# awslabs/flowgger

Hardware: NVIDIA H100
Metric: log lines/sec parsed (RFC5424) (higher is better)
Workload: dtype u8

## Files before the change

### flowgger_b200/csrc/fg_abi.cu

```cuda
#include <cuda_runtime.h>

#include <algorithm>
#include <chrono>
#include <cstdio>
#include <cstdlib>
#include <cstring>
#include <ctime>
#include <mutex>
#include <new>
#include <string>
#include <utility>
#include <vector>

#include "../../include/flowgger_cuda.h"
#include "fg_kernels.cuh"
#include "fg_status.h"
#include "fg_rfc3164.cuh"
#include "fg_tz.h"

namespace {

const char* kErrorStrings[FG_ST_COUNT] = {};
struct ErrorTableInit {
    ErrorTableInit() {
// ... 90 lines not shown
    H h = nullptr;
    Handle() = default;
    Handle(Handle&& o) noexcept : h(o.h) { o.h = nullptr; }
    Handle(const Handle&) = delete;
    Handle& operator=(const Handle&) = delete;
    ~Handle() {
        if (h) destroy(h);
    }
    operator H() const { return h; }
};
using Event = Handle<cudaEvent_t>;
using Stream = Handle<cudaStream_t>;

struct StepEvents {
    Event h2d;
    Event k0, k1;
    Event cnt;
};

enum { T_ENTRIES, T_E8, T_ARENA, T_WIDE, T_COUNT };
struct TableShape {
    size_t width[3];
    size_t round;
};
constexpr TableShape kTableShape[T_COUNT] = {
    {{sizeof(fg_span), sizeof(uint64_t), 1}, 256},
    {{sizeof(uint64_t), 0, 0}, 256},
    {{1, 0, 0}, 256},
    {{sizeof(fg_wide_row), 0, 0}, 1},
};
static_assert(sizeof(fg_span) == sizeof(int2) && sizeof(fg_wide_row) == sizeof(fg::WideRow), "pinned rows mirror the device rows");
struct Table {
    Buf<uint8_t> col[3];
    size_t cap = 0;
};

struct TableUse {
    int table, counter;
    size_t div, floor;
    bool grow;
};
struct FormatTables {
    int n;
    TableUse use[4];
    const TableUse* begin() const { return use; }
    const TableUse* end() const { return use + n; }
};
constexpr FormatTables kFormatTables[4] = {
    {4, {{T_E8, fg::K5_ENTRIES, 24, 4096, false}, {T_ARENA, fg::K5_ARENA, 64, 64 << 10, false},
         {T_WIDE, fg::K5_WIDE_ROWS, 0, 1024, false}, {T_ENTRIES, fg::K5_WIDE_ENTRIES, 0, 4096, false}}},
    {1, {{T_ENTRIES, fg::K5_ENTRIES, 24, 4096, true}}},
    {1, {{T_ENTRIES, fg::K5_ENTRIES, 24, 4096, true}}},
    {2, {{T_ARENA, fg::K5_ARENA, 32, 64 << 10, false}, {T_ENTRIES, -1, 0, 256, false}}},
};

}

struct fg_ctx {
    int device = 0;
    size_t max_bytes = 0;
    int max_lines = 0;
    int chunk_lines = 0;
    int input_format = 0;
    Stream s_h2d, s_comp, s_d2h;
    Stream s_parse;
    Event ev_a, ev_b;
    Event ev_dom0, ev_dom1;
    Event ev_s0, ev_s1;
    std::vector<StepEvents> steps;
    std::vector<Event> ev_split;
    Event bounce_ev[2];
    Buf<uint8_t> bounce[2];
    Buf<uint32_t> counts;
    Buf<uint8_t> bytes;
    Buf<int32_t> offsets;
    Buf<uint32_t> k;
    Buf<uint8_t> flush;
    Table tab[T_COUNT];
    Buf<uint8_t> rows;
    Buf<int2> tmp_name;
    Buf<unsigned long long> tmp_val;
    Buf<uint8_t> tmp_meta;
    Buf<fg::Row5424, fg_row5424> rows5;
    Buf<uint32_t> esc_list, wide_list;
    Buf<unsigned long long> enc_lens, enc_rel;
    Buf<unsigned long long> enc_base;
    Buf<uint8_t> enc_out;
    size_t enc_out_cap = 0;
    Buf<long long, int64_t> enc_offsets;
    Buf<uint8_t> enc_status;
    Buf<int32_t> enc_stop;
    int enc_stop_n = -1;
    Buf<uint8_t> scan_temp;
    size_t scan_temp_bytes = 0;
    Buf<uint8_t> static_blob;
    int n_static = 0;
    const int32_t* d_static_key_off = nullptr;
    const int32_t* d_static_lit_off = nullptr;
    const int32_t* d_static_kind = nullptr;
    std::vector<std::pair<std::string, std::string>> gelf_extra;
    Buf<uint32_t> seg;
    Buf<int32_t> n_lines;
    Buf<uint8_t> invalid;
    Buf<int32_t> split_offsets;
    Buf<int32_t> cum;
    float last_split_ms = 0.f;
    int r3164_year = 0;
    int call_year = 1970;
    std::string tzdir;
    fg::TzHostTable tz_host;
    Buf<uint8_t> tz_blob;
    fg::TzDeviceTable tz_dev{};
    Buf<uint8_t> ltsv_blob;
    fg::LtsvDeviceConfig ltsv{};
    float last_dom_ms = 0.f;
    int res_n = 0;
    size_t res_bytes = 0;
    int res_fmt = -1;
    uint32_t res_tot[fg::K5_COUNT] = {};
    std::string last_error;
    int64_t launches = 0;
    int max_tile5 = 0;
    int num_sms = 0;
};

namespace {

constexpr int kColW[9] = {8, 4, 8, 8, 8, 8, 8, 8, 8};
enum { C_TS = 0, C_META, C_HOST, C_APP, C_PROC, C_MSGID, C_MSG, C_FULL, C_SD, C_COUNT };
size_t col_off(const fg_ctx* c, int col) {
    const size_t n = (size_t)c->max_lines;
    size_t o = 0;
    for (int k = 0; k < col; ++k) o += (size_t)kColW[k] * n;
    return o;
}

int fail(fg_ctx* c, int code, const char* what, cudaError_t e = cudaSuccess) {
    if (c) {
        c->last_error = what;
        if (e != cudaSuccess) {
            c->last_error += ": ";
            c->last_error += cudaGetErrorString(e);
        }
    }
    return code;
}

#define FG_CUDA(ctx, call)                                         \
    do {                                                           \
        cudaError_t _e = (call);                                   \
        if (_e != cudaSuccess) return fail(ctx, FG_E_CUDA, #call, _e); \
    } while (0)

cudaError_t create(Event& e, unsigned flags) { return cudaEventCreateWithFlags(&e.h, flags); }
cudaError_t create(Stream& s) { return cudaStreamCreateWithFlags(&s.h, cudaStreamNonBlocking); }

template <class T>
T* dev(const fg_ctx* c, int t, int col = 0) {
    return reinterpret_cast<T*>(c->tab[t].col[col].d);
}
template <class T>
T* host(const fg_ctx* c, int t, int col = 0) {
    return reinterpret_cast<T*>(c->tab[t].col[col].h);
}
uint32_t cap32(const fg_ctx* c, int t) { return (uint32_t)std::min<size_t>(c->tab[t].cap, 0xFFFFFFFFu); }

int grow_table(fg_ctx* c, int t, size_t rows) {
// ... 38 lines not shown
    std::vector<uint8_t> bytes;
    template <class V>
    size_t add(const V& v) {
        const size_t at = bytes.size();
        const uint8_t* src = reinterpret_cast<const uint8_t*>(v.data());
        bytes.insert(bytes.end(), src, src + v.size() * sizeof(v[0]));
        bytes.resize((bytes.size() + 15) & ~(size_t)15, 0);
        return at;
    }
    int upload(fg_ctx* c, Buf<uint8_t>& blob) {
        bytes.resize(bytes.size() + 16, 0);
        FG_CUDA(c, blob.alloc(bytes.size(), DEV));
        FG_CUDA(c, cudaMemcpy(blob.d, bytes.data(), bytes.size(), cudaMemcpyHostToDevice));
        return FG_OK;
    }
};

int upload_tz(fg_ctx* c) {
    const fg::TzHostTable& H = c->tz_host;
    Packer p;
    const size_t o_hash = p.add(H.hash), o_key = p.add(H.key), o_zone = p.add(H.zone), o_noff = p.add(H.name_off),
                 o_first = p.add(H.first), o_off = p.add(H.off), o_names = p.add(H.names);
    if (int rc = p.upload(c, c->tz_blob)) return rc;
    const uint8_t* b = c->tz_blob.d;
    fg::TzDeviceTable& T = c->tz_dev;
    T = H.view();
    T.hash = (const unsigned long long*)(b + o_hash);
    T.key = (const long long*)(b + o_key);
    T.zone = (const int32_t*)(b + o_zone);
    T.name_off = (const int32_t*)(b + o_noff);
    T.first = (const int32_t*)(b + o_first);
    T.off = (const int32_t*)(b + o_off);
    T.names = b + o_names;
    return FG_OK;
}

int upload_ltsv_config(fg_ctx* c, const fg_config* cfg) {
    std::vector<uint8_t> names, suffix;
    std::vector<int32_t> name_off{0}, types;
    const int ns = (cfg->ltsv_schema_names && cfg->ltsv_schema_types) ? cfg->ltsv_schema_len : 0;
    for (int k = 0; k < ns; ++k) {
        const char* s = cfg->ltsv_schema_names[k];
        names.insert(names.end(), (const uint8_t*)s, (const uint8_t*)s + strlen(s));
        name_off.push_back((int32_t)names.size());
        types.push_back(cfg->ltsv_schema_types[k]);
    }
    fg::LtsvDeviceConfig& L = c->ltsv;
    L.has_schema = (cfg->ltsv_has_schema || ns > 0) ? 1 : 0;
    L.n_schema = ns;
    L.suffix_present = 0;
    L.suffix_off[0] = 0;
    for (int t = 0; t < 5; ++t) {
        const char* s = cfg->ltsv_suffix[t];
        if (t > 0 && s) {
            L.suffix_present |= 1u << t;
            suffix.insert(suffix.end(), (const uint8_t*)s, (const uint8_t*)s + strlen(s));
        }
        L.suffix_off[t + 1] = (int32_t)suffix.size();
    }
    Packer p;
    const size_t o_names = p.add(names), o_off = p.add(name_off), o_types = p.add(types), o_suf = p.add(suffix);
    if (int rc = p.upload(c, c->ltsv_blob)) return rc;
    const uint8_t* b = c->ltsv_blob.d;
    L.names = b + o_names;
    L.name_off = (const int32_t*)(b + o_off);
    L.types = (const int32_t*)(b + o_types);
    L.suffix = b + o_suf;
    return FG_OK;
}

int current_year(const fg_ctx* c) {
    if (c->r3164_year != 0) return c->r3164_year;
    const time_t now = time(nullptr);
    struct tm g;
    gmtime_r(&now, &g);
    return g.tm_year + 1900;
}

int ensure_format(fg_ctx* c, int fmt) {
    const size_t L = (size_t)c->max_lines;
    if (fmt == FG_FMT_RFC5424) {
        if (!c->rows5.d) {
            FG_CUDA(c, c->rows5.alloc(L, BOTH));
            FG_CUDA(c, c->esc_list.alloc(L, DEV));
            FG_CUDA(c, c->wide_list.alloc(L, DEV));
        }
    } else if (!c->rows.d) {
        FG_CUDA(c, c->rows.alloc(col_off(c, C_COUNT), BOTH));
    }
    if (fmt == FG_FMT_GELF && !c->wide_list.d) FG_CUDA(c, c->wide_list.alloc(L, DEV));
    for (const TableUse& u : kFormatTables[fmt]) {
        const size_t first = u.div ? std::max<size_t>(c->max_bytes / u.div, u.floor) : u.floor;
        const size_t cap = c->tab[u.table].cap;
        if (u.grow ? cap < first : !cap)
            if (int rc = grow_table(c, u.table, first)) return rc;
    }
    if (fmt == FG_FMT_RFC3164) {
        if (!c->tz_host.loaded) {
            std::string err;
            if (!fg::tz_load_dir(c->tzdir.empty() ? nullptr : c->tzdir.c_str(), c->tz_host, err)) return fail(c, FG_E_ARG, err.c_str());
        }
        if (!c->tz_blob.d)
            if (int rc = upload_tz(c)) return rc;
    }
    if (fmt == FG_FMT_LTSV || fmt == FG_FMT_GELF) {
        const size_t need = (fmt == FG_FMT_LTSV ? c->max_bytes / 2 + L : c->max_bytes / 3) + 64;
        if (c->tmp_meta.n < need) {
            c->tmp_name.reset(); c->tmp_val.reset(); c->tmp_meta.reset();
            FG_CUDA(c, c->tmp_name.alloc(need, DEV));
            FG_CUDA(c, c->tmp_val.alloc(need, DEV));
            FG_CUDA(c, c->tmp_meta.alloc(need, DEV));
        }
    }
    return FG_OK;
}

int begin_call(fg_ctx* c, fg_format fmt) {
    if ((int)fmt < 0 || (int)fmt > 3) return fail(c, FG_E_ARG, "unknown format");
    FG_CUDA(c, cudaSetDevice(c->device));
    if (int rc = ensure_format(c, (int)fmt)) return rc;
    c->call_year = current_year(c);
    return FG_OK;
}

int pick_tile(const fg_ctx* c, size_t total_bytes, int n, int fmt) {
    const double mean = n > 0 ? (double)total_bytes / n : 0.0;
    const long lines = fg::lines_per_cta(fmt), gran = 8 * lines;
    const int max_tile[4] = {c->max_tile5, fg::kLtsvMaxTile, fg::kGelfMaxTile, fg::kR3164MaxTile};
    long t = (long)(mean * lines * 1.02) + gran;
    t = (t + gran - 1) / gran * gran;
    t = std::max(t, 8L * 1024);
    t = std::min(t, (long)max_tile[fmt]);
    return (int)t;
}

int launch_lines(fg_ctx* c, int fmt, int line0, int n, int tile, const uint8_t* invalid, int strip_eol, cudaStream_t s,
                 bool time_dominant = false) {
    if (fmt == FG_FMT_RFC5424) {
        fg::Parse5424Params P;
        P.bytes = c->bytes.d;
        P.offsets = c->offsets.d + line0;
        P.n = n;
        P.tile_bytes = tile;
        P.rows = reinterpret_cast<uint4*>(c->rows5.d + line0);
        P.entries = dev<unsigned long long>(c, T_E8);
        P.entry_cap = cap32(c, T_E8);
        P.counters = c->k.d;
        P.esc_list = c->esc_list.d;
        P.wide_list = c->wide_list.d;
        P.arena = dev<uint8_t>(c, T_ARENA);
        P.arena_cap = cap32(c, T_ARENA);
        P.wide_rows = dev<fg::WideRow>(c, T_WIDE);
        P.wide_cap = cap32(c, T_WIDE);
        P.wentry_name = dev<int2>(c, T_ENTRIES, 0);
        P.wentry_val = dev<unsigned long long>(c, T_ENTRIES, 1);
        P.wentry_meta = dev<uint8_t>(c, T_ENTRIES, 2);
        P.wentry_cap = cap32(c, T_ENTRIES);
        P.line0 = line0;
        P.bad_offsets = c->k.d + fg::K5_BAD_OFFSETS;
        P.line_invalid = invalid;
        P.strip_eol = strip_eol;
        P.num_sms = c->num_sms;
        FG_CUDA(c, cudaMemsetAsync(c->k.d + fg::K5_ESC_LIST, 0, 8, s));
        FG_CUDA(c, fg::launch_parse5424(P, s, time_dominant ? c->ev_dom0.h : nullptr, time_dominant ? c->ev_dom1.h : nullptr));
        c->launches += 2;
        return FG_OK;
    }
    fg::ParseParams P;
    P.bytes = c->bytes.d;
    P.offsets = c->offsets.d + line0;
    P.n = n;
    P.line0 = line0;
    P.tile_bytes = tile;
    P.num_sms = c->num_sms;
    uint8_t* r = c->rows.d;
    P.ts = (double*)(r + col_off(c, C_TS)) + line0;
    P.meta = (uint32_t*)(r + col_off(c, C_META)) + line0;
    P.host = (int2*)(r + col_off(c, C_HOST)) + line0;
    P.app = (int2*)(r + col_off(c, C_APP)) + line0;
    P.proc = (int2*)(r + col_off(c, C_PROC)) + line0;
    P.msgid = (int2*)(r + col_off(c, C_MSGID)) + line0;
    P.msg = (int2*)(r + col_off(c, C_MSG)) + line0;
    P.full = (int2*)(r + col_off(c, C_FULL)) + line0;
    P.sd = (int2*)(r + col_off(c, C_SD)) + line0;
    P.entry_name = dev<int2>(c, T_ENTRIES, 0);
    P.entry_val = dev<unsigned long long>(c, T_ENTRIES, 1);
    P.entry_meta = dev<uint8_t>(c, T_ENTRIES, 2);
    P.tmp_name = c->tmp_name.d;
    P.tmp_val = c->tmp_val.d;
    P.tmp_meta = c->tmp_meta.d;
    P.line_invalid = invalid;
    P.strip_eol = strip_eol;
    P.entry_counter = c->k.d + fg::K5_ENTRIES;
    P.entry_cap = cap32(c, T_ENTRIES);
    P.bad_offsets = c->k.d + fg::K5_BAD_OFFSETS;
    P.slow_list = c->wide_list.d;
    P.slow_count = c->k.d + fg::K5_WIDE_LIST;
    if (fmt == FG_FMT_GELF) FG_CUDA(c, cudaMemsetAsync(c->k.d + fg::K5_WIDE_LIST, 0, 4, s));
    P.ltsv = c->ltsv;
    P.r3164.year = c->call_year;
    P.r3164.tz = c->tz_dev;
    P.r3164.arena = dev<uint8_t>(c, T_ARENA);
    P.r3164.arena_cap = cap32(c, T_ARENA);
    P.r3164.arena_counter = c->k.d + fg::K5_ARENA;
    if (time_dominant) FG_CUDA(c, cudaEventRecord(c->ev_dom0, s));
    FG_CUDA(c, fg::launch_parse(fmt, P, s));
    if (time_dominant) FG_CUDA(c, cudaEventRecord(c->ev_dom1, s));
    c->launches += fmt == FG_FMT_GELF ? 2 : 1;
    return FG_OK;
}

bool gelf_fusable(const fg_ctx* c, int fmt) {
    return fmt == FG_FMT_RFC5424 || fmt == FG_FMT_RFC3164 || (fmt == FG_FMT_LTSV && c->input_format == FG_FMT_LTSV);
}

int launch_encode(fg_ctx* c, int fmt, int k, int l0, int n, int tile, cudaStream_t s) {
    fg::GelfEncodeParams E{};
    E.bytes = c->bytes.d;
    E.offsets = c->offsets.d + l0;
    E.n = n;
    if (fmt == FG_FMT_RFC5424) {
        E.rows = reinterpret_cast<const uint4*>(c->rows5.d + l0);
    } else {
        const uint8_t* r = c->rows.d;
        E.col_ts = (const double*)(r + col_off(c, C_TS)) + l0;
        E.col_meta = (const uint32_t*)(r + col_off(c, C_META)) + l0;
        E.col_host = (const int2*)(r + col_off(c, C_HOST)) + l0;
        E.col_msg = (const int2*)(r + col_off(c, C_MSG)) + l0;
        E.col_full = (const int2*)(r + col_off(c, C_FULL)) + l0;
    }
    if (fmt == FG_FMT_LTSV) {
        E.col_sd = (const int2*)(c->rows.d + col_off(c, C_SD)) + l0;
        E.ltsv_suffix = c->ltsv.suffix;
        for (int t = 0; t < 6; ++t) E.ltsv_suffix_off[t] = c->ltsv.suffix_off[t];
        E.ltsv_stop = c->enc_stop.d + l0;
    }
    E.entries = dev<unsigned long long>(c, T_E8);
    E.arena = dev<uint8_t>(c, T_ARENA);
    E.wide_rows = dev<fg::WideRow>(c, T_WIDE);
    E.wentry_name = dev<int2>(c, T_ENTRIES, 0);
    E.wentry_val = dev<unsigned long long>(c, T_ENTRIES, 1);
    E.wentry_meta = dev<uint8_t>(c, T_ENTRIES, 2);
    E.static_blob = c->static_blob.d;
    E.n_static = c->n_static;
    E.static_key_off = c->d_static_key_off;
    E.static_lit_off = c->d_static_lit_off;
// ... 855 lines not shown
```

### flowgger_b200/csrc/fg_kernels.cuh

```cuda
#pragma once
#include <stdint.h>
#ifdef FG_HOST_EMU
#include "../../tests/emu/cuda_shim.h"
#else
#include <cuda_runtime.h>
#endif

namespace fg {

struct LtsvDeviceConfig {
    int32_t has_schema;
    int32_t n_schema;
    const uint8_t* names;
    const int32_t* name_off;
    const int32_t* types;
    const uint8_t* suffix;
    int32_t suffix_off[6];
    uint32_t suffix_present;
};

struct TzDeviceTable {
    int32_t n_names;
    int32_t min_len, max_len;
    uint32_t first_mask[8];
    const unsigned long long* hash;
    const int32_t* zone;
    const int32_t* name_off;
    const uint8_t* names;
    const int32_t* first;
    const long long* key;
    const int32_t* off;
};
struct R3164DeviceConfig {
    int32_t year;
    TzDeviceTable tz;
    uint8_t* arena;
    uint32_t arena_cap;
    uint32_t* arena_counter;
};

struct ParseParams {
    const uint8_t* bytes;
    const int32_t* offsets;
    int32_t n;
    int32_t line0;
    int32_t tile_bytes;
    double* ts;
    uint32_t* meta;
    int2* host;
    int2* app;
    int2* proc;
    int2* msgid;
    int2* msg;
    int2* full;
    int2* sd;
    int2* entry_name;
    unsigned long long* entry_val;
    uint8_t* entry_meta;
    int2* tmp_name;
    unsigned long long* tmp_val;
    uint8_t* tmp_meta;
    const uint8_t* line_invalid;
    int32_t strip_eol;
    uint32_t* entry_counter;
    uint32_t entry_cap;
    const uint32_t* bad_offsets;
    uint32_t* slow_list;
    uint32_t* slow_count;
    int32_t num_sms;
    LtsvDeviceConfig ltsv;
    R3164DeviceConfig r3164;
};

struct Row5424 {
    double ts;
    uint32_t meta;
    uint32_t sd_first;
    uint16_t sd_count;
    uint16_t sp[5];
    uint16_t msg_off, msg_len;
};
static_assert(sizeof(Row5424) == 32, "Row5424 must be 32 bytes");
struct WideRow {
    int32_t line;
    uint32_t meta;
    double ts;
    int2 host, app, proc, msgid, msg, full, sd;
};
static_assert(sizeof(WideRow) == 72, "WideRow must be 72 bytes");

enum { K5_ENTRIES = 0, K5_ARENA = 1, K5_WIDE_ROWS = 2, K5_WIDE_ENTRIES = 3, K5_ESC_LIST = 4, K5_WIDE_LIST = 5, K5_BAD_OFFSETS = 6,
       K5_COUNT = 8 };

struct Parse5424Params {
    const uint8_t* bytes;
    const int32_t* offsets;
    int32_t n;
    int32_t tile_bytes;
    uint4* rows;
    unsigned long long* entries;
    uint32_t entry_cap;
    uint32_t* counters;
    uint32_t* esc_list;
    uint32_t* wide_list;
    uint8_t* arena;
    uint32_t arena_cap;
    WideRow* wide_rows;
    uint32_t wide_cap;
    int2* wentry_name;
    unsigned long long* wentry_val;
    uint8_t* wentry_meta;
    uint32_t wentry_cap;
    int32_t line0;
    const uint32_t* bad_offsets;
    const uint8_t* line_invalid;
    int32_t strip_eol;
    int32_t num_sms;
};

cudaError_t launch_parse5424(const Parse5424Params& p, cudaStream_t stream, cudaEvent_t dom0 = nullptr, cudaEvent_t dom1 = nullptr);
cudaError_t configure_parse5424(int max_tile_bytes);
int parse5424_smem_bytes(int tile_bytes);

struct GelfEncodeParams {
    const uint8_t* bytes;
    const int32_t* offsets;
    int32_t n;
    const uint4* rows;
    const unsigned long long* entries;
    const uint8_t* arena;
    const WideRow* wide_rows;
    const int2* wentry_name;
    const unsigned long long* wentry_val;
    const uint8_t* wentry_meta;
    const uint8_t* static_blob;
    int32_t n_static;
    const int32_t* static_key_off;
    const int32_t* static_lit_off;
    const int32_t* static_kind;
    unsigned long long* lens;
    unsigned long long* rel;
    unsigned long long* base;
    uint8_t* out;
    unsigned long long out_cap;
    long long* out_offsets;
    uint8_t* status;
    const uint32_t* bad_offsets;
    uint32_t entry_cap, wide_cap, wentry_cap;
    int32_t tile_bytes;
    const double* col_ts;
    const uint32_t* col_meta;
    const int2* col_host;
    const int2* col_msg;
    const int2* col_full;
    uint32_t arena_cap;
    const int2* col_sd;
    const uint8_t* ltsv_suffix;
    int32_t ltsv_suffix_off[6];
    int32_t* ltsv_stop;
};
cudaError_t configure_gelf_encode(int max_tile_bytes);
cudaError_t launch_gelf_encode(int fmt, const GelfEncodeParams& p, void* d_scan_temp, size_t scan_temp_bytes, cudaStream_t stream);
size_t gelf_scan_temp_bytes(int n);

#ifndef FG_R5_LINES
#define FG_R5_LINES 64
#endif
#ifndef FG_R5_MINB
#define FG_R5_MINB 16
#endif
constexpr int kRfc5424LinesPerCta = FG_R5_LINES;
constexpr int kRfc5424CtasPerSm = FG_R5_MINB;
#ifndef FG_LTSV_LINES
#define FG_LTSV_LINES 64
#endif
#ifndef FG_LTSV_THREADS
#define FG_LTSV_THREADS 256
#endif
constexpr int kLtsvLinesPerCta = FG_LTSV_LINES;
constexpr int kLtsvThreadsPerCta = FG_LTSV_THREADS;
constexpr int kLtsvStageSlots = kLtsvLinesPerCta * 24;
constexpr int kLtsvMaxTile = 65024;
#ifndef FG_GELF_LINES
#define FG_GELF_LINES 64
#endif
#ifndef FG_GELF_THREADS
// ... 43 lines not shown
```

### flowgger_b200/csrc/fg_parse5424.cu

```cuda
#include "fg_kernels.cuh"

#include "fg_common.cuh"
#include "fg_r5fast.cuh"
#include "fg_rfc5424.cuh"
#include "fg_status.h"
#include "fg_tma.cuh"

namespace fg {

namespace {

constexpr int kFastLines = kRfc5424LinesPerCta;
constexpr int kFastCtasPerSm = kRfc5424CtasPerSm;

template <int LINES, int MINB>
__global__ void __launch_bounds__(LINES, MINB) parse5424_kernel(const __grid_constant__ Parse5424Params P) {
    extern __shared__ __align__(128) uint8_t tile[];
    __shared__ __align__(8) uint64_t mbar;
    __shared__ uint32_t scan_ws[2 * (LINES / 32)];
    __shared__ uint32_t s_base[3];

    const int tid = threadIdx.x;
    const uint32_t lane = (uint32_t)tid & 31u;
    const int first = blockIdx.x * LINES;
    const int last = min(P.n, first + LINES);
    uint32_t* bmI = reinterpret_cast<uint32_t*>(tile + P.tile_bytes);
    if (*P.bad_offsets) return;
    if (tid == 0) mbar_init(&mbar, 1);
    __syncthreads();

    uint32_t parity = 0;
    int cur = first;
    while (cur < last) {
        const int i = cur + tid;
        const int o0 = __ldg(P.offsets + min(i, last));
        const int o1 = __ldg(P.offsets + min(i + 1, last));
        const int ocur = __ldg(P.offsets + cur);
        const int base = ocur & ~15;
        const bool fits = (i < last) && (o1 - base <= P.tile_bytes);
        const int r = __syncthreads_count(fits);
        if (r == 0) {
            if (tid == 0) P.wide_list[atomicAdd(P.counters + K5_WIDE_LIST, 1u)] = (uint32_t)cur;
            cur += 1;
            continue;
        }
        const int oend = __ldg(P.offsets + cur + r);
        const uint32_t nbytes = (uint32_t)((oend - base) + 15) & ~15u;
        if (tid == 0) {
            fence_proxy_async();
            mbar_expect_tx(&mbar, nbytes);
            bulk_g2s(tile, P.bytes + base, nbytes, &mbar);
        }
        mbar_wait(&mbar, parity);
        parity ^= 1u;

        const int nword = (int)((nbytes + 31u) >> 5);
        for (int g = tid; g < nword; g += LINES) {
            const uint4 v0 = reinterpret_cast<const uint4*>(tile)[2 * g], v1 = reinterpret_cast<const uint4*>(tile)[2 * g + 1];
            bmI[g] = r5_classify16(v0.x, v0.y, v0.z, v0.w) | (r5_classify16(v1.x, v1.y, v1.z, v1.w) << 16);
        }
        if (tid < 3) bmI[nword + tid] = 0;
        __syncthreads();

        const bool active = tid < r;
        int ls = active ? o0 - base : 0;
        int le = active ? o1 - base : 0;
        bool bad_utf8 = false;
        if (P.strip_eol && le > ls) {
            if (P.strip_eol == 2) {
                if (tile[le - 1] == 0) --le;
            } else if (tile[le - 1] == '\n') {
                --le;
                if (le > ls && tile[le - 1] == '\r') --le;
            }
            if (P.line_invalid != nullptr && P.line_invalid[i]) bad_utf8 = true;
        }
        const bool too_long = le - ls > 65535;
        R5Fast res;
        const bool regular = r5_regular(tile, bmI, ls, (too_long || bad_utf8 || !active) ? ls : le, res);
        if (bad_utf8) {
            res.status = FG_ES_INVALID_UTF8;
            res.n_entries = 0;
        }
        const bool wide = active && !regular && !bad_utf8;
        const uint32_t my_n = (active && !wide && res.status == FG_ST_OK) ? res.n_entries : 0u;
        const bool esc = my_n != 0u && res.esc;

        uint32_t xa = my_n, xb = (esc ? 1u : 0u) | (wide ? 0x100u : 0u);
#pragma unroll
        for (int d = 1; d < 32; d <<= 1) {
            const uint32_t ya = __shfl_up_sync(0xFFFFFFFFu, xa, d), yb = __shfl_up_sync(0xFFFFFFFFu, xb, d);
            if (lane >= (uint32_t)d) { xa += ya; xb += yb; }
        }
        const int wid = tid >> 5;
        constexpr int kWarps = LINES / 32;
        if (lane == 31u) { scan_ws[wid] = xa; scan_ws[kWarps + wid] = xb; }
        __syncthreads();
        uint32_t before_a = 0, before_b = 0, total = 0, total_b = 0;
#pragma unroll
        for (int w = 0; w < kWarps; ++w) {
            const uint32_t ta = scan_ws[w], tb = scan_ws[kWarps + w];
            if (w < wid) { before_a += ta; before_b += tb; }
            total += ta;
            total_b += tb;
        }
        const uint32_t excl = before_a + xa - my_n;
        const uint32_t pos_b = before_b + xb - ((esc ? 1u : 0u) | (wide ? 0x100u : 0u));
        const uint32_t n_esc = total_b & 0xFFu, n_wide = total_b >> 8;
        if (total | total_b) {
            if (tid == 0 && total) s_base[0] = atomicAdd(P.counters + K5_ENTRIES, total);
            if (tid == 32 % LINES && n_esc) s_base[1] = atomicAdd(P.counters + K5_ESC_LIST, n_esc);
            if (tid == 33 % LINES && n_wide) s_base[2] = atomicAdd(P.counters + K5_WIDE_LIST, n_wide);
            __syncthreads();
        }
        const uint32_t esc_at = pos_b & 0xFFu, wide_at = pos_b >> 8;
        uint32_t my_begin = 0;
        if (my_n) {
            my_begin = s_base[0] + excl;
            if ((unsigned long long)my_begin + my_n <= (unsigned long long)P.entry_cap) {
                unsigned long long* dst = P.entries + my_begin;
                for (uint32_t k = 0; k < my_n; ++k) dst[k] = res.stage[k];
            }
        }
        if (esc) P.esc_list[s_base[1] + esc_at] = (uint32_t)i;
        if (wide) P.wide_list[s_base[2] + wide_at] = (uint32_t)i;
        if (active && !wide) {
            const bool ok = res.status == FG_ST_OK;
            const uint32_t meta = ok ? (res.facility << 8) | (res.severity << 16) | (res.flags << 24) : res.status | 0x00FFFF00u;
            uint4 lo4, hi4;
            lo4.x = (uint32_t)__double2loint(res.ts);
            lo4.y = (uint32_t)__double2hiint(res.ts);
            lo4.z = meta;
            lo4.w = my_begin;
            hi4.x = my_n | ((uint32_t)res.sp1 << 16);
            hi4.y = (uint32_t)res.sp2 | ((uint32_t)res.sp3 << 16);
            hi4.z = (uint32_t)res.sp4 | ((uint32_t)res.sp5 << 16);
            hi4.w = (uint32_t)res.msg_o | ((uint32_t)res.msg_l << 16);
            if (!ok) {
                lo4.x = lo4.y = 0u;
                hi4 = make_uint4(0u, 0u, 0u, 0u);
            }
            P.rows[2 * (size_t)i] = lo4;
            P.rows[2 * (size_t)i + 1] = hi4;
        }
        __syncthreads();
        cur += r;
    }
}

__device__ __forceinline__ void unescape_lines(const Parse5424Params& P, uint32_t first_item, uint32_t stride) {
    const uint32_t cnt = P.counters[K5_ESC_LIST];
    const uint32_t lane = threadIdx.x & 31u;
    for (uint32_t j0 = first_item; j0 < cnt; j0 += stride) {
        const uint32_t j = j0 + lane;
        const bool valid = j < cnt;
        uint32_t first = 0, count = 0;
        int o0 = 0;
        if (valid) {
            const uint32_t line = P.esc_list[j];
            const uint4 lo4 = P.rows[2 * (size_t)line], hi4 = P.rows[2 * (size_t)line + 1];
            o0 = P.offsets[line];
            first = lo4.w;
            count = hi4.x & 0xFFFFu;
            if ((unsigned long long)first + count > (unsigned long long)P.entry_cap) count = 0;
        }
        uint32_t need = 0;
        for (uint32_t e = 0; e < count; ++e) {
            const unsigned long long v = P.entries[first + e];
            if (!(v & kE8Header) && (v & kE8Esc)) need += (2u + (uint32_t)((v >> 32) & 0xFFFFu) - ((uint32_t)((v >> 16) & 0xFFFFu) + 2u) + 1u) & ~1u;
        }
        uint32_t inc = need;
#pragma unroll
        for (int d = 1; d < 32; d <<= 1) {
            const uint32_t y = __shfl_up_sync(0xFFFFFFFFu, inc, d);
            if (lane >= (uint32_t)d) inc += y;
        }
        const uint32_t warp_total = __shfl_sync(0xFFFFFFFFu, inc, 31);
        uint32_t abase = 0;
        if (lane == 0 && warp_total) abase = atomicAdd(P.counters + K5_ARENA, warp_total);
        abase = __shfl_sync(0xFFFFFFFFu, abase, 0);
        if ((unsigned long long)abase + warp_total > (unsigned long long)P.arena_cap) continue;
        uint32_t at = abase + inc - need;
        uint32_t e = 0;
        for (;;) {
            unsigned long long v = 0;
            bool have = false;
            for (; e < count; ++e) {
                v = P.entries[first + e];
                if (!(v & kE8Header) && (v & kE8Esc)) { have = true; break; }
            }
            if (!__any_sync(0xFFFFFFFFu, have)) break;
            const int ne = (int)((v >> 16) & 0xFFFFu), ve = (int)((v >> 32) & 0xFFFFu);
            const int len = have ? ve - (ne + 2) : 0;
            const uint8_t* src = P.bytes + o0 + ne + 2;
            uint8_t* dst = P.arena + at + 2;
            int k = 0, o = 0;
            while (__any_sync(0xFFFFFFFFu, k < len)) {
                if (k < len) {
                    const uint32_t c = src[k++];
                    if (c != '\\') {
                        dst[o++] = (uint8_t)c;
                    } else if (k < len) {
                        const uint32_t d = src[k++];
                        if (d != '"' && d != '\\' && d != ']') dst[o++] = '\\';
                        dst[o++] = (uint8_t)d;
                    }
                }
            }
            if (have) {
                *reinterpret_cast<uint16_t*>(P.arena + at) = (uint16_t)o;
                P.entries[first + e] = (v & 0xFFFFFFFFull) | ((unsigned long long)(at >> 1) << 32) | kE8Arena;
                at += (2u + (uint32_t)len + 1u) & ~1u;
                ++e;
            }
        }
    }
}

__device__ __forceinline__ void wide_lines(const Parse5424Params& P, int (*marks)[32], uint32_t first_item, uint32_t stride) {
    const uint32_t cnt = P.counters[K5_WIDE_LIST];
    const uint32_t lane = threadIdx.x & 31u;
    const EntrySink sink = {P.wentry_name, P.wentry_val, P.wentry_meta};
    for (uint32_t j0 = first_item; j0 < cnt; j0 += stride) {
        const uint32_t j = j0 + lane;
        const bool valid = j < cnt;
        uint32_t line = 0;
        int o0 = 0, len = 0;
        bool bad_utf8 = false;
        if (valid) {
            line = P.wide_list[j];
            o0 = P.offsets[line];
            len = P.offsets[line + 1] - o0;
            if (P.strip_eol && len > 0) {
                if (P.strip_eol == 2) {
                    if (P.bytes[o0 + len - 1] == 0) --len;
                } else if (P.bytes[o0 + len - 1] == '\n') {
                    --len;
                    if (len > 0 && P.bytes[o0 + len - 1] == '\r') --len;
                }
                if (P.line_invalid != nullptr && P.line_invalid[line]) bad_utf8 = true;
            }
            if (bad_utf8) len = 0;
        }
        LineResult res;
        rfc5424_parse_line<32>(P.bytes + o0, len, o0, &marks[0][lane], res, sink, 0u, false);
        uint32_t n = (valid && !bad_utf8 && res.status == FG_ST_OK) ? res.n_entries : 0u;
        uint32_t wbase = 0;
        if (n) {
            wbase = atomicAdd(P.counters + K5_WIDE_ENTRIES, n);
            if ((unsigned long long)wbase + n > (unsigned long long)P.wentry_cap) n = 0;
        }
        {
            LineResult again;
            rfc5424_parse_line<32>(P.bytes + o0, n ? len : 0, o0, &marks[0][lane], again, sink, wbase, true);
        }
        if (!valid) continue;
        for (uint32_t k = 0; k < n; ++k) {
            const uint32_t e = wbase + k;
            const uint8_t m = sink.meta[e];
            if ((m & 0x07u) == 0u && (m & 0x08u)) {
                const unsigned long long v = sink.val[e];
                const uint32_t off = (uint32_t)v, l = (uint32_t)(v >> 32);
                const uint32_t ul = (uint32_t)r5_unescape(P.bytes + off, (int)l, nullptr);
                const uint32_t at = atomicAdd(P.counters + K5_ARENA, (ul + 1u) & ~1u);
                if ((unsigned long long)at + ul <= (unsigned long long)P.arena_cap) r5_unescape(P.bytes + off, (int)l, P.arena + at);
                sink.val[e] = (unsigned long long)at | ((unsigned long long)ul << 32);
                sink.meta[e] = (uint8_t)0x80u;
            }
        }
        if (bad_utf8) {
            res.status = FG_ES_INVALID_UTF8;
            res.flags = 0;
            res.facility = res.severity = 0xFFu;
        }
        const bool ok = res.status == FG_ST_OK;
        if (!ok) {
            P.rows[2 * (size_t)line] = make_uint4(0u, 0u, res.status | 0x00FFFF00u, 0u);
            P.rows[2 * (size_t)line + 1] = make_uint4(0u, 0u, 0u, 0u);
            continue;
        }
        const uint32_t widx = atomicAdd(P.counters + K5_WIDE_ROWS, 1u);
        const uint32_t meta = res.status | (res.facility << 8) | (res.severity << 16) | ((res.flags | kFlagWide) << 24);
        if (widx < P.wide_cap) {
            WideRow w;
            w.line = P.line0 + (int32_t)line;
            w.meta = meta;
            w.ts = res.ts;
            w.host = make_int2(ok ? o0 + res.host_o : -1, res.host_l);
            w.app = make_int2(ok ? o0 + res.app_o : -1, res.app_l);
            w.proc = make_int2(ok ? o0 + res.proc_o : -1, res.proc_l);
            w.msgid = make_int2(ok ? o0 + res.mid_o : -1, res.mid_l);
            w.msg = make_int2(ok && res.msg_o >= 0 ? o0 + res.msg_o : -1, res.msg_l);
            w.full = make_int2(ok && res.full_o >= 0 ? o0 + res.full_o : -1, res.full_l);
            w.sd = make_int2((int)wbase, (int)(ok ? n : 0u));
            P.wide_rows[widx] = w;
        }
        P.rows[2 * (size_t)line] = make_uint4((uint32_t)__double2loint(res.ts), (uint32_t)__double2hiint(res.ts), meta, widx);
        P.rows[2 * (size_t)line + 1] = make_uint4(0u, 0u, 0u, 0u);
    }
}

__global__ void __launch_bounds__(128) post5424_kernel(const __grid_constant__ Parse5424Params P, int esc_ctas) {
    __shared__ int marks[4][6][32];
    if (*P.bad_offsets) return;
    const uint32_t warp = threadIdx.x >> 5;
    if ((int)blockIdx.x < esc_ctas) {
        unescape_lines(P, (blockIdx.x * 4u + warp) * 32u, (uint32_t)esc_ctas * 128u);
    } else {
        const uint32_t wctas = gridDim.x - (uint32_t)esc_ctas;
        wide_lines(P, marks[warp], ((blockIdx.x - (uint32_t)esc_ctas) * 4u + warp) * 32u, wctas * 128u);
    }
}

}

int parse5424_smem_bytes(int tile_bytes) { return tile_bytes + tile_bytes / 8 + 16; }

cudaError_t configure_parse5424(int max_tile_bytes) {
    return cudaFuncSetAttribute(parse5424_kernel<kFastLines, kFastCtasPerSm>, cudaFuncAttributeMaxDynamicSharedMemorySize,
                                parse5424_smem_bytes(max_tile_bytes));
}

cudaError_t launch_parse5424(const Parse5424Params& p, cudaStream_t stream, cudaEvent_t dom0, cudaEvent_t dom1) {
    if (p.n <= 0) return cudaSuccess;
    const int grid = (p.n + kFastLines - 1) / kFastLines;
    if (dom0) cudaEventRecord(dom0, stream);
    parse5424_kernel<kFastLines, kFastCtasPerSm><<<grid, kFastLines, parse5424_smem_bytes(p.tile_bytes), stream>>>(p);
    if (dom1) cudaEventRecord(dom1, stream);
    const long long sms = p.num_sms;
    const int esc_ctas = (int)min((long long)(p.n + 127) / 128, sms * 12);
    const int wide_ctas = (int)min((long long)(p.n + 127) / 128, sms * 4);
    post5424_kernel<<<esc_ctas + wide_ctas, 128, 0, stream>>>(p, esc_ctas);
    return cudaGetLastError();
}

}
```

### flowgger_b200/csrc/fg_r5fast.cuh

```cuda
#pragma once
#include "fg_common.cuh"
#include "fg_status.h"

namespace fg {

FG_DEV uint32_t r5_flags(uint32_t w) {
    const uint32_t low = w & 0x7F7F7F7Fu;
    const uint32_t a2 = low + 0x5D5D5D5Du;
    const uint32_t a1 = low + 0x01010101u;
    const uint32_t x = (w & 0x1E1E1E1Eu) ^ 0x1C1C1C1Cu;
    const uint32_t a3 = x + 0x7F7F7F7Fu;
    return (~a2 | a1 | w | ~a3) & 0x80808080u;
}
FG_DEV uint32_t r5_nibble_top(uint32_t f) { return f * 0x00204081u; }
FG_DEV uint32_t r5_gather16(uint32_t f0, uint32_t f1, uint32_t f2, uint32_t f3) {
    const uint32_t n0 = r5_nibble_top(f0), n1 = r5_nibble_top(f1), n2 = r5_nibble_top(f2), n3 = r5_nibble_top(f3);
    return (n0 >> 28) | ((n1 >> 24) & 0xF0u) | ((n2 >> 20) & 0xF00u) | ((n3 >> 16) & 0xF000u);
}
FG_DEV uint32_t r5_classify16(uint32_t w0, uint32_t w1, uint32_t w2, uint32_t w3) {
    return r5_gather16(r5_flags(w0), r5_flags(w1), r5_flags(w2), r5_flags(w3));
}
FG_DEV uint32_t r5_window(const uint32_t* bm, int t) {
    const int k = t >> 5;
    return fg_funnel_r(bm[k], bm[k + 1], (uint32_t)t & 31u);
}

constexpr unsigned long long kE8Esc = 1ull << 48;
constexpr unsigned long long kE8Header = 1ull << 63;
constexpr unsigned long long kE8Arena = 1ull << 62;
FG_DEV unsigned long long r5_pack_pair8(int ns, int ne, int ve, bool esc) {
    return (unsigned long long)(uint32_t)ns | ((unsigned long long)(uint32_t)ne << 16) | ((unsigned long long)(uint32_t)ve << 32) |
           (esc ? kE8Esc : 0ull);
}
FG_DEV unsigned long long r5_pack_header8(int es, int id_end, uint32_t pairs) {
    return (unsigned long long)(uint32_t)es | ((unsigned long long)(uint32_t)id_end << 16) | ((unsigned long long)(pairs & 0xFFFFu) << 32) | kE8Header;
}

struct R5Fast {
    double ts;
    uint32_t status, facility, severity, flags;
    int sp1, sp2, sp3, sp4, sp5;
    int msg_o, msg_l;
    uint32_t n_entries;
    unsigned long long* stage;
    bool esc;
};

FG_DEV int r5_unescape(const uint8_t* v, int len, uint8_t* out) {
    int o = 0;
    bool esc = false;
    for (int k = 0; k < len; ++k) {
        const uint8_t c = v[k];
        if (!esc) {
            if (c == '\\') esc = true;
            else {
                if (out) out[o] = c;
                ++o;
            }
        } else {
            if (c != '"' && c != '\\' && c != ']') {
                if (out) out[o] = '\\';
                ++o;
            }
            if (out) out[o] = c;
            ++o;
            esc = false;
        }
    }
    return o;
}

FG_DEV int r5_unescape_to(const uint8_t* v, int len, uint8_t* out) {
    int o = 0;
    for (int k = 0; k < len; ++k) {
        const uint32_t c = v[k];
        if (c != '\\') {
            out[o++] = (uint8_t)c;
        } else if (k + 1 < len) {
            const uint32_t d = v[++k];
            if (d != '"' && d != '\\' && d != ']') out[o++] = '\\';
            out[o++] = (uint8_t)d;
        }
    }
    return o;
}

constexpr uint32_t kFlagWide = 0x80u;

FG_DEV uint32_t r5_digit(const uint8_t* T, int at, uint32_t& worst) {
    const uint32_t d = (uint32_t)T[at] - (uint32_t)'0';
    worst = max(worst, d);
    return d;
}

FG_DEV bool r5_regular(uint8_t* T, const uint32_t* bmI, int ls, int le, R5Fast& r) {
    r.ts = 0.0;
    r.status = FG_ST_OK;
    r.facility = 0xFFu;
    r.severity = 0xFFu;
    r.flags = 0;
    r.sp1 = r.sp2 = r.sp3 = r.sp4 = r.sp5 = 0;
    r.msg_o = r.msg_l = 0;
    r.n_entries = 0;
    r.stage = nullptr;
    r.esc = false;
    bool ok = le - ls >= 32;

    int sp[6];
    {
        int t = ls + 1;
#pragma unroll
        for (int k = 0; k < 6; ++k) {
            uint32_t W = r5_window(bmI, t);
            if (k == 1 && W == 0u) {
                t += 32;
                W = r5_window(bmI, t);
            }
            t += fg_ffs(W) - 1;
            ok = ok && W != 0u && t < le && T[t] == ' ';
            sp[k] = t;
            t = ok ? t + 1 : ls;
        }
    }
    uint32_t bad = 0;
    {
        const int l0 = sp[0] - ls;
        ok = ok && T[ls] == '<' && l0 >= 4 && l0 <= 6;
        const int gt = ok ? sp[0] - 2 : ls;
        ok = ok && T[gt] == '>' && T[gt + 1] == '1';
        uint32_t pri = 0;
        for (int q = ls + 1; q < gt; ++q) pri = pri * 10u + r5_digit(T, q, bad);
        ok = ok && pri <= 255u;
        r.facility = pri >> 3;
        r.severity = pri & 7u;
    }
    {
        const int a = ok ? sp[0] + 1 : ls, e = ok ? sp[1] : ls;
        const int L = e - a;
        ok = ok && L >= 20;
        const int z = ok ? e - 1 : ls;
        const bool zulu = T[z] == 'Z';
        const int zone = zulu ? z : z - 5;
        DateTime t;
        t.year = (int)(r5_digit(T, a, bad) * 1000u + r5_digit(T, a + 1, bad) * 100u + r5_digit(T, a + 2, bad) * 10u + r5_digit(T, a + 3, bad));
        t.month = (int)(r5_digit(T, a + 5, bad) * 10u + r5_digit(T, a + 6, bad));
        t.day = (int)(r5_digit(T, a + 8, bad) * 10u + r5_digit(T, a + 9, bad));
        t.hour = (int)(r5_digit(T, a + 11, bad) * 10u + r5_digit(T, a + 12, bad));
        t.minute = (int)(r5_digit(T, a + 14, bad) * 10u + r5_digit(T, a + 15, bad));
        t.second = (int)(r5_digit(T, a + 17, bad) * 10u + r5_digit(T, a + 18, bad));
        ok = ok && T[a + 4] == '-' && T[a + 7] == '-' && T[a + 10] == 'T' && T[a + 13] == ':' && T[a + 16] == ':';
        const int fl = zone - (a + 19);
        ok = ok && (fl == 0 || (fl >= 2 && fl <= 10 && T[a + 19] == '.'));
        uint32_t nanos = 0, mult = 100000000u;
#pragma unroll
        for (int k = 0; k < 9; ++k) {
            if (k + 1 < fl) nanos += r5_digit(T, a + 20 + k, bad) * mult;
            mult /= 10u;
        }
        t.nanos = nanos;
        int off = 0;
        if (!zulu) {
            const uint32_t sg = T[zone];
            const int oh = (int)(r5_digit(T, zone + 1, bad) * 10u + r5_digit(T, zone + 2, bad));
            const int om = (int)(r5_digit(T, zone + 4, bad) * 10u + r5_digit(T, zone + 5, bad));
            ok = ok && (sg == '+' || sg == '-') && T[zone + 3] == ':' && oh <= 23 && om <= 59 && zone >= a + 19;
            off = oh * 3600 + om * 60;
            if (sg == '-') off = -off;
        }
        t.offset_seconds = off;
        ok = ok && bad <= 9u && t.second <= 59;
        if (!ok) { t.year = 2000; t.month = 1; t.day = 1; t.hour = t.minute = t.second = 0; t.nanos = 0; t.offset_seconds = 0; }
        double ts = 0.0;
        ok = finish_datetime(t, false, ts) && ok;
        r.ts = ts;
    }
    fg_syncwarp();

    const int d = ok ? sp[5] + 1 : ls;
    int msg_from = le;
    bool walk = false;
    ok = ok && d < le;
    if (ok) {
        const uint32_t c0 = T[d];
        if (c0 == '-') msg_from = d + 1;
        else if (c0 == '[') walk = true;
        else ok = false;
    }
    {
        const int sbase = (ls + 7) & ~7;
        unsigned long long* stg = (unsigned long long*)(T + sbase);
        uint32_t n = 0, pairs = 0, hdr = 0;
        int i = d + 1, elem_start = 0, id_end = 0;
        bool st_id = true, active = walk, any_esc = false;
        while (fg_any(active)) {
            if (active && st_id) {
                const uint32_t W = r5_window(bmI, i);
                const int s1 = i + fg_ffs(W) - 1;
                if (W == 0u || s1 >= le || T[s1] != ' ') { ok = false; active = false; }
                else { elem_start = i; id_end = s1; i = s1 + 1; st_id = false; hdr = n++; pairs = 0; }
            }
            int e = i;
            if (active) {
                const uint32_t W = r5_window(bmI, i);
                e = i + fg_ffs(W) - 1;
                if (W == 0u || (W & 1u) || e + 2 >= le || T[e] != '=' || T[e + 1] != '"') { ok = false; active = false; }
            }
            int c = e + 2;
            bool has_bs = false;
            {
                bool s = active;
                for (;;) {
                    if (s) {
                        uint32_t W = r5_window(bmI, c);
                        const int room = le - c;
                        if (room < 32) W &= (1u << room) - 1u;
                        int adv = 32;
                        while (W) {
                            const int b = fg_ffs(W) - 1;
                            const uint32_t ch = T[c + b];
                            if (ch == '"') { adv = b; s = false; break; }
                            W &= W - 1u;
                            if (ch == '\\') {
                                has_bs = true;
                                W &= ~(2u << b);
                                if (b == 31) adv = 33;
                            }
                        }
                        c += adv;
                        if (s && c >= le) { c = le; s = false; }
                    }
                    if (!fg_any(s)) break;
                }
            }
            if (active) {
                if (c + 1 >= le || sbase + 8 * ((int)n + 1) > c + 1) { ok = false; active = false; }
                else {
                    stg[n++] = r5_pack_pair8(i - ls, e - ls, c - ls, has_bs);
                    any_esc |= has_bs;
                    ++pairs;
                    const uint32_t nx = T[c + 1];
                    if (nx == ' ') {
                        i = c + 2;
                        if (i >= le) { ok = false; active = false; }
                    } else if (nx == ']') {
                        stg[hdr] = r5_pack_header8(elem_start - ls, id_end - ls, pairs);
                        const uint32_t n2 = c + 2 < le ? T[c + 2] : 0u;
                        if (n2 == ' ') { msg_from = c + 2; active = false; }
                        else if (n2 == '[') { i = c + 3; st_id = true; }
                        else { ok = false; active = false; }
                    } else { ok = false; active = false; }
                }
            }
        }
        if (walk && ok) {
            r.n_entries = n;
            r.stage = stg;
            r.esc = any_esc;
        }
    }

    int hi = le, lo = msg_from;
    {
        bool plain_end = true, plain_start = true;
        if (ok) {
            const uint32_t cl = T[le - 1];
            plain_end = cl > 0x20u && cl < 0x80u;
            plain_start = false;
            if (msg_from + 1 < le) {
                const uint32_t c0 = T[msg_from], c1 = T[msg_from + 1];
                plain_start = c0 == ' ' && c1 > 0x20u && c1 < 0x80u;
            }
        }
        if (fg_any(!plain_end)) {
            if (ok && !plain_end) hi = trim_end(T, msg_from, le);
        }
        if (fg_any(!plain_start)) {
            if (ok) lo = plain_start ? msg_from + 1 : trim_start(T, msg_from, hi);
        } else {
            lo = msg_from + 1;
        }
    }
    if (ok) {
        if (hi > lo) {
            r.msg_o = lo - ls;
            r.msg_l = hi - lo;
        } else {
            r.msg_o = msg_from - ls;
            r.msg_l = 0;
        }
        r.sp1 = sp[1] - ls;
        r.sp2 = sp[2] - ls;
        r.sp3 = sp[3] - ls;
        r.sp4 = sp[4] - ls;
        r.sp5 = sp[5] - ls;
    }
    fg_syncwarp();
    return ok;
}

}
```

Baseline: 6.708 billion.

## Fuse SD-value unescaping into the RFC5424 parse kernel using the shared tile

Removes the separate escape-list pass in the post kernel. Arena space is now reserved in the parse kernel through the existing warp scan and atomic. Escaped structured-data values are unescaped directly from the shared-memory tile, using a warp-cooperative ballot/bitmask unescape. A slower serial path reading global bytes is used when the staging area overlaps the source. This avoids a second global read of entries and bytes and reduces post-kernel grid work, at the cost of extra work and registers in the main parse kernel.

```diff
diff --git a/flowgger_b200/csrc/fg_abi.cu b/flowgger_b200/csrc/fg_abi.cu
--- a/flowgger_b200/csrc/fg_abi.cu
+++ b/flowgger_b200/csrc/fg_abi.cu
@@ -196,7 +196,7 @@
     Buf<unsigned long long> tmp_val;
     Buf<uint8_t> tmp_meta;
     Buf<fg::Row5424, fg_row5424> rows5;
-    Buf<uint32_t> esc_list, wide_list;
+    Buf<uint32_t> wide_list;
     Buf<unsigned long long> enc_lens, enc_rel;
     Buf<unsigned long long> enc_base;
     Buf<uint8_t> enc_out;
@@ -401,7 +401,6 @@
     if (fmt == FG_FMT_RFC5424) {
         if (!c->rows5.d) {
             FG_CUDA(c, c->rows5.alloc(L, BOTH));
-            FG_CUDA(c, c->esc_list.alloc(L, DEV));
             FG_CUDA(c, c->wide_list.alloc(L, DEV));
         }
     } else if (!c->rows.d) {
@@ -465,7 +464,6 @@
         P.entries = dev<unsigned long long>(c, T_E8);
         P.entry_cap = cap32(c, T_E8);
         P.counters = c->k.d;
-        P.esc_list = c->esc_list.d;
         P.wide_list = c->wide_list.d;
         P.arena = dev<uint8_t>(c, T_ARENA);
         P.arena_cap = cap32(c, T_ARENA);
@@ -480,7 +478,7 @@
         P.line_invalid = invalid;
         P.strip_eol = strip_eol;
         P.num_sms = c->num_sms;
-        FG_CUDA(c, cudaMemsetAsync(c->k.d + fg::K5_ESC_LIST, 0, 8, s));
+        FG_CUDA(c, cudaMemsetAsync(c->k.d + fg::K5_WIDE_LIST, 0, 4, s));
         FG_CUDA(c, fg::launch_parse5424(P, s, time_dominant ? c->ev_dom0.h : nullptr, time_dominant ? c->ev_dom1.h : nullptr));
         c->launches += 2;
         return FG_OK;
diff --git a/flowgger_b200/csrc/fg_kernels.cuh b/flowgger_b200/csrc/fg_kernels.cuh
--- a/flowgger_b200/csrc/fg_kernels.cuh
+++ b/flowgger_b200/csrc/fg_kernels.cuh
@@ -89,8 +89,7 @@
 };
 static_assert(sizeof(WideRow) == 72, "WideRow must be 72 bytes");
 
-enum { K5_ENTRIES = 0, K5_ARENA = 1, K5_WIDE_ROWS = 2, K5_WIDE_ENTRIES = 3, K5_ESC_LIST = 4, K5_WIDE_LIST = 5, K5_BAD_OFFSETS = 6,
-       K5_COUNT = 8 };
+enum { K5_ENTRIES = 0, K5_ARENA = 1, K5_WIDE_ROWS = 2, K5_WIDE_ENTRIES = 3, K5_WIDE_LIST = 4, K5_BAD_OFFSETS = 5, K5_COUNT = 8 };
 
 struct Parse5424Params {
     const uint8_t* bytes;
@@ -101,7 +100,6 @@
     unsigned long long* entries;
     uint32_t entry_cap;
     uint32_t* counters;
-    uint32_t* esc_list;
     uint32_t* wide_list;
     uint8_t* arena;
     uint32_t arena_cap;
diff --git a/flowgger_b200/csrc/fg_parse5424.cu b/flowgger_b200/csrc/fg_parse5424.cu
--- a/flowgger_b200/csrc/fg_parse5424.cu
+++ b/flowgger_b200/csrc/fg_parse5424.cu
@@ -12,6 +12,57 @@
 
 constexpr int kFastLines = kRfc5424LinesPerCta;
 constexpr int kFastCtasPerSm = kRfc5424CtasPerSm;
+
+__device__ __forceinline__ void unescape_from_tile(uint8_t* tile, const uint8_t* gtile, uint8_t* arena, bool esc, bool buried, int ls,
+                                                   uint32_t n, uint32_t at) {
+    const uint32_t lane = threadIdx.x & 31u;
+    const uint32_t below = (1u << lane) - 1u;
+    if (buried) {
+        unsigned long long* stg = reinterpret_cast<unsigned long long*>(tile + ((ls + 7) & ~7));
+        for (uint32_t k = 0; k < n; ++k) {
+            const unsigned long long v = stg[k];
+            if ((v & (kE8Header | kE8Esc)) != kE8Esc) continue;
+            const int vs = ls + (int)((v >> 16) & 0xFFFFu) + 2, len = ls + (int)((v >> 32) & 0xFFFFu) - vs;
+            *reinterpret_cast<uint16_t*>(arena + at) = (uint16_t)r5_unescape_to(gtile + vs, len, arena + at + 2u);
+            stg[k] = (v & 0xFFFFFFFFull) | ((unsigned long long)(at >> 1) << 32) | kE8Arena;
+            at += (2u + (uint32_t)len + 1u) & ~1u;
+        }
+    }
+    for (uint32_t todo = __ballot_sync(0xFFFFFFFFu, esc && !buried); todo; todo &= todo - 1u) {
+        const int src = __ffs(todo) - 1;
+        const int l_ls = __shfl_sync(0xFFFFFFFFu, ls, src);
+        const uint32_t l_n = __shfl_sync(0xFFFFFFFFu, n, src);
+        uint32_t l_at = __shfl_sync(0xFFFFFFFFu, at, src);
+        unsigned long long* stg = reinterpret_cast<unsigned long long*>(tile + ((l_ls + 7) & ~7));
+        for (uint32_t k0 = 0; k0 < l_n; k0 += 32u) {
+            const uint32_t k = k0 + lane;
+            const unsigned long long v = k < l_n ? stg[k] : 0ull;
+            for (uint32_t pend = __ballot_sync(0xFFFFFFFFu, (v & (kE8Header | kE8Esc)) == kE8Esc); pend; pend &= pend - 1u) {
+                const int j = __ffs(pend) - 1;
+                const unsigned long long vj = __shfl_sync(0xFFFFFFFFu, v, j);
+                const int vs = l_ls + (int)((vj >> 16) & 0xFFFFu) + 2;
+                const int len = l_ls + (int)((vj >> 32) & 0xFFFFu) - vs;
+                uint8_t* dst = arena + l_at + 2u;
+                uint32_t carry = 0, o = 0;
+                for (int q = 0; q < len; q += 32) {
+                    const int left = len - q;
+                    const uint32_t valid = left >= 32 ? 0xFFFFFFFFu : (1u << left) - 1u;
+                    const uint32_t c = tile[vs + q + (int)lane];
+                    const uint32_t after = tile[vs + q + min(left, 32)];
+                    const uint32_t keep = r5_unescape_keep(__ballot_sync(0xFFFFFFFFu, c == '\\'),
+                                                           __ballot_sync(0xFFFFFFFFu, c == '"' || c == '\\' || c == ']'), valid,
+                                                           after != '"' && after != '\\' && after != ']', carry);
+                    if ((keep >> lane) & 1u) dst[o + __popc(keep & below)] = (uint8_t)c;
+                    o += __popc(keep);
+                }
+                if (lane == 0u) *reinterpret_cast<uint16_t*>(arena + l_at) = (uint16_t)o;
+                if (lane == (uint32_t)j) stg[k] = (v & 0xFFFFFFFFull) | ((unsigned long long)(l_at >> 1) << 32) | kE8Arena;
+                l_at += (2u + (uint32_t)len + 1u) & ~1u;
+            }
+        }
+    }
+    __syncwarp();
+}
 
 template <int LINES, int MINB>
 __global__ void __launch_bounds__(LINES, MINB) parse5424_kernel(const __grid_constant__ Parse5424Params P) {
@@ -85,8 +136,10 @@
         const bool wide = active && !regular && !bad_utf8;
         const uint32_t my_n = (active && !wide && res.status == FG_ST_OK) ? res.n_entries : 0u;
         const bool esc = my_n != 0u && res.esc;
-
-        uint32_t xa = my_n, xb = (esc ? 1u : 0u) | (wide ? 0x100u : 0u);
+        const uint32_t my_arena = esc ? res.esc_need : 0u;
+
+        const uint32_t my_b = my_arena | (wide ? 1u << 24 : 0u);
+        uint32_t xa = my_n, xb = my_b;
 #pragma unroll
         for (int d = 1; d < 32; d <<= 1) {
             const uint32_t ya = __shfl_up_sync(0xFFFFFFFFu, xa, d), yb = __shfl_up_sync(0xFFFFFFFFu, xb, d);
@@ -105,15 +158,17 @@
             total_b += tb;
         }
         const uint32_t excl = before_a + xa - my_n;
-        const uint32_t pos_b = before_b + xb - ((esc ? 1u : 0u) | (wide ? 0x100u : 0u));
-        const uint32_t n_esc = total_b & 0xFFu, n_wide = total_b >> 8;
+        const uint32_t pos_b = before_b + xb - my_b;
+        const uint32_t n_arena = total_b & 0xFFFFFFu, n_wide = total_b >> 24;
         if (total | total_b) {
             if (tid == 0 && total) s_base[0] = atomicAdd(P.counters + K5_ENTRIES, total);
-            if (tid == 32 % LINES && n_esc) s_base[1] = atomicAdd(P.counters + K5_ESC_LIST, n_esc);
+            if (tid == 32 % LINES && n_arena) s_base[1] = atomicAdd(P.counters + K5_ARENA, n_arena);
             if (tid == 33 % LINES && n_wide) s_base[2] = atomicAdd(P.counters + K5_WIDE_LIST, n_wide);
             __syncthreads();
         }
-        const uint32_t esc_at = pos_b & 0xFFu, wide_at = pos_b >> 8;
+        if (n_arena && (unsigned long long)s_base[1] + n_arena <= (unsigned long long)P.arena_cap)
+            unescape_from_tile(tile, P.bytes + base, P.arena, esc, esc && r5_esc_buried(ls, res), ls, my_n, s_base[1] + (pos_b & 0xFFFFFFu));
+        const uint32_t wide_at = pos_b >> 24;
         uint32_t my_begin = 0;
         if (my_n) {
             my_begin = s_base[0] + excl;
@@ -122,7 +177,6 @@
                 for (uint32_t k = 0; k < my_n; ++k) dst[k] = res.stage[k];
             }
         }
-        if (esc) P.esc_list[s_base[1] + esc_at] = (uint32_t)i;
         if (wide) P.wide_list[s_base[2] + wide_at] = (uint32_t)i;
         if (active && !wide) {
             const bool ok = res.status == FG_ST_OK;
@@ -145,75 +199,6 @@
         }
         __syncthreads();
         cur += r;
-    }
-}
-
-__device__ __forceinline__ void unescape_lines(const Parse5424Params& P, uint32_t first_item, uint32_t stride) {
-    const uint32_t cnt = P.counters[K5_ESC_LIST];
-    const uint32_t lane = threadIdx.x & 31u;
-    for (uint32_t j0 = first_item; j0 < cnt; j0 += stride) {
-        const uint32_t j = j0 + lane;
-        const bool valid = j < cnt;
-        uint32_t first = 0, count = 0;
-        int o0 = 0;
-        if (valid) {
-            const uint32_t line = P.esc_list[j];
-            const uint4 lo4 = P.rows[2 * (size_t)line], hi4 = P.rows[2 * (size_t)line + 1];
-            o0 = P.offsets[line];
-            first = lo4.w;
-            count = hi4.x & 0xFFFFu;
-            if ((unsigned long long)first + count > (unsigned long long)P.entry_cap) count = 0;
-        }
-        uint32_t need = 0;
-        for (uint32_t e = 0; e < count; ++e) {
-            const unsigned long long v = P.entries[first + e];
-            if (!(v & kE8Header) && (v & kE8Esc)) need += (2u + (uint32_t)((v >> 32) & 0xFFFFu) - ((uint32_t)((v >> 16) & 0xFFFFu) + 2u) + 1u) & ~1u;
-        }
-        uint32_t inc = need;
-#pragma unroll
-        for (int d = 1; d < 32; d <<= 1) {
-            const uint32_t y = __shfl_up_sync(0xFFFFFFFFu, inc, d);
-            if (lane >= (uint32_t)d) inc += y;
-        }
-        const uint32_t warp_total = __shfl_sync(0xFFFFFFFFu, inc, 31);
-        uint32_t abase = 0;
-        if (lane == 0 && warp_total) abase = atomicAdd(P.counters + K5_ARENA, warp_total);
-        abase = __shfl_sync(0xFFFFFFFFu, abase, 0);
-        if ((unsigned long long)abase + warp_total > (unsigned long long)P.arena_cap) continue;
-        uint32_t at = abase + inc - need;
-        uint32_t e = 0;
-        for (;;) {
-            unsigned long long v = 0;
-            bool have = false;
-            for (; e < count; ++e) {
-                v = P.entries[first + e];
-                if (!(v & kE8Header) && (v & kE8Esc)) { have = true; break; }
-            }
-            if (!__any_sync(0xFFFFFFFFu, have)) break;
-            const int ne = (int)((v >> 16) & 0xFFFFu), ve = (int)((v >> 32) & 0xFFFFu);
-            const int len = have ? ve - (ne + 2) : 0;
-            const uint8_t* src = P.bytes + o0 + ne + 2;
-            uint8_t* dst = P.arena + at + 2;
-            int k = 0, o = 0;
-            while (__any_sync(0xFFFFFFFFu, k < len)) {
-                if (k < len) {
-                    const uint32_t c = src[k++];
-                    if (c != '\\') {
-                        dst[o++] = (uint8_t)c;
-                    } else if (k < len) {
-                        const uint32_t d = src[k++];
-                        if (d != '"' && d != '\\' && d != ']') dst[o++] = '\\';
-                        dst[o++] = (uint8_t)d;
-                    }
-                }
-            }
-            if (have) {
-                *reinterpret_cast<uint16_t*>(P.arena + at) = (uint16_t)o;
-                P.entries[first + e] = (v & 0xFFFFFFFFull) | ((unsigned long long)(at >> 1) << 32) | kE8Arena;
-                at += (2u + (uint32_t)len + 1u) & ~1u;
-                ++e;
-            }
-        }
     }
 }
 
@@ -300,16 +285,11 @@
     }
 }
 
-__global__ void __launch_bounds__(128) post5424_kernel(const __grid_constant__ Parse5424Params P, int esc_ctas) {
+__global__ void __launch_bounds__(128) post5424_kernel(const __grid_constant__ Parse5424Params P) {
     __shared__ int marks[4][6][32];
     if (*P.bad_offsets) return;
     const uint32_t warp = threadIdx.x >> 5;
-    if ((int)blockIdx.x < esc_ctas) {
-        unescape_lines(P, (blockIdx.x * 4u + warp) * 32u, (uint32_t)esc_ctas * 128u);
-    } else {
-        const uint32_t wctas = gridDim.x - (uint32_t)esc_ctas;
-        wide_lines(P, marks[warp], ((blockIdx.x - (uint32_t)esc_ctas) * 4u + warp) * 32u, wctas * 128u);
-    }
+    wide_lines(P, marks[warp], (blockIdx.x * 4u + warp) * 32u, gridDim.x * 128u);
 }
 
 }
@@ -327,10 +307,8 @@
     if (dom0) cudaEventRecord(dom0, stream);
     parse5424_kernel<kFastLines, kFastCtasPerSm><<<grid, kFastLines, parse5424_smem_bytes(p.tile_bytes), stream>>>(p);
     if (dom1) cudaEventRecord(dom1, stream);
-    const long long sms = p.num_sms;
-    const int esc_ctas = (int)min((long long)(p.n + 127) / 128, sms * 12);
-    const int wide_ctas = (int)min((long long)(p.n + 127) / 128, sms * 4);
-    post5424_kernel<<<esc_ctas + wide_ctas, 128, 0, stream>>>(p, esc_ctas);
+    const int wide_ctas = (int)min((long long)(p.n + 127) / 128, (long long)p.num_sms * 4);
+    post5424_kernel<<<wide_ctas, 128, 0, stream>>>(p);
     return cudaGetLastError();
 }
 
diff --git a/flowgger_b200/csrc/fg_r5fast.cuh b/flowgger_b200/csrc/fg_r5fast.cuh
--- a/flowgger_b200/csrc/fg_r5fast.cuh
+++ b/flowgger_b200/csrc/fg_r5fast.cuh
@@ -44,6 +44,8 @@
     uint32_t n_entries;
     unsigned long long* stage;
     bool esc;
+    uint32_t esc_need;
+    int esc_from;
 };
 
 FG_DEV int r5_unescape(const uint8_t* v, int len, uint8_t* out) {
@@ -83,6 +85,17 @@
         }
     }
     return o;
+}
+
+FG_DEV uint32_t r5_unescape_keep(uint32_t bs, uint32_t sp, uint32_t valid, uint32_t next_plain, uint32_t& carry) {
+    constexpr uint32_t kEven = 0x55555555u;
+    const uint32_t b = bs & valid & ~carry;
+    const uint32_t starts = b & ~(b << 1);
+    const uint32_t run_even = b & ~(b + (starts & kEven)), run_odd = b & ~(b + (starts & ~kEven));
+    const uint32_t escaping = (run_even & kEven) | (run_odd & ~kEven);
+    carry = escaping >> 31;
+    const uint32_t plain_after = ((valid & ~sp) >> 1) | (next_plain << 31);
+    return valid & ~(escaping & ~plain_after);
 }
 
 constexpr uint32_t kFlagWide = 0x80u;
@@ -104,6 +117,8 @@
     r.n_entries = 0;
     r.stage = nullptr;
     r.esc = false;
+    r.esc_need = 0;
+    r.esc_from = 0;
     bool ok = le - ls >= 32;
 
     int sp[6];
@@ -189,9 +204,9 @@
     {
         const int sbase = (ls + 7) & ~7;
         unsigned long long* stg = (unsigned long long*)(T + sbase);
-        uint32_t n = 0, pairs = 0, hdr = 0;
-        int i = d + 1, elem_start = 0, id_end = 0;
-        bool st_id = true, active = walk, any_esc = false;
+        uint32_t n = 0, pairs = 0, hdr = 0, esc_need = 0;
+        int i = d + 1, elem_start = 0, id_end = 0, esc_from = 0;
+        bool st_id = true, active = walk;
         while (fg_any(active)) {
             if (active && st_id) {
                 const uint32_t W = r5_window(bmI, i);
@@ -236,7 +251,10 @@
                 if (c + 1 >= le || sbase + 8 * ((int)n + 1) > c + 1) { ok = false; active = false; }
                 else {
                     stg[n++] = r5_pack_pair8(i - ls, e - ls, c - ls, has_bs);
-                    any_esc |= has_bs;
+                    if (has_bs) {
+                        if (esc_need == 0u) esc_from = e + 2;
+                        esc_need += (2u + (uint32_t)(c - (e + 2)) + 1u) & ~1u;
+                    }
                     ++pairs;
                     const uint32_t nx = T[c + 1];
                     if (nx == ' ') {
@@ -255,7 +273,9 @@
         if (walk && ok) {
             r.n_entries = n;
             r.stage = stg;
-            r.esc = any_esc;
+            r.esc = esc_need != 0u;
+            r.esc_need = esc_need;
+            r.esc_from = esc_from;
         }
     }
 
@@ -298,4 +318,8 @@
     return ok;
 }
 
-}
+FG_DEV bool r5_esc_buried(int ls, const R5Fast& r) {
+    return r.esc && r.esc_from < ((ls + 7) & ~7) + 8 * (int)r.n_entries;
+}
+
+}
```

Measured after the change: 6.943 billion, median of 6. 3.5% higher.
